# vfdev-5/interpolate-antialiasing

Hardware: AMD Instinct MI355X
Metric: Mpix/s (input pixels) antialiased bilinear 438x906->196x320, uint8 channels_last, PIL-exact (higher is better)
Workload: dtype u8; 1 GPU; uint8 channels_last [1024,3,438,906]->[196,320] bilinear antialias per GPU (BASELINE configs[1] batched), Pillow-exact integer arithmetic; batch_per_gpu=1024, global_batch=1024, variant=fused_u8_nhwc_pil_v3, parallelism=batch-shard x1, lib=interpolate_antialiasing_amd/csrc/libaa_interp.so

## Files before the change

interpolate_antialiasing_amd/csrc/aa_fused_u8_v3_impl.h:

```cpp

#pragma once
#include <math.h>
#include <stdio.h>
#include <stdlib.h>

#include <type_traits>

#include "aa_alpha.h"
#include "aa_plan.h"

#ifndef AA_V3_ABL
#define AA_V3_ABL 0
#endif

#ifndef AA_V3_AUX
#define AA_V3_AUX 0
#endif

#ifndef AA_V3_PRIO
#define AA_V3_PRIO 0
#endif
#ifndef AA_V3_DMA_EARLY
#define AA_V3_DMA_EARLY 0
#endif

#ifndef AA_V3_BURST
#define AA_V3_BURST 1
#endif

#ifndef AA_V3_F32OUT_AUX
#define AA_V3_F32OUT_AUX 0
#endif

#ifndef AA_V3_FLT_FAST
#define AA_V3_FLT_FAST 0
#endif

#ifndef AA_V3_UNALIGNED
#define AA_V3_UNALIGNED 0
#endif

struct FusedU8V3Params {
  int H, W, oH, oW;
  int ksize_w, ksize_h;
  int ybands, nstrips;
  int strips_per_block;
  int strip_w;
  int nseg;
  int seg_bytes;
  int sc_off;
  int gather_off;
  int in_mis;
  unsigned long long img_in_bytes, img_out_bytes, total_in_bytes, total_out_bytes;
  long long n_images;
  int spb_forced;
  int outm, normalize, cin;
  float mean[4], std[4];
  unsigned row_pitch;
  int fast;
  int byte_store;
  unsigned long long plane_in_bytes, plane_out_bytes;
  long long pl_planes;
  int out16, pair_store;
};

namespace {

typedef __attribute__((address_space(3))) void lds_void;

#ifndef AA_V3_STORE_AUX
#define AA_V3_STORE_AUX 2
#endif
constexpr int kStoreAuxInterleaved = AA_V3_STORE_AUX;




__device__ inline unsigned pack2_bf16(float lo, float hi) {
  unsigned d;
  asm("v_cvt_pk_bf16_f32 %0, %1, %2" : "=v"(d) : "v"(lo), "v"(hi));
  return d;
}
__device__ inline unsigned pack2_f16(float lo, float hi) {
  typedef _Float16 half2_t __attribute__((ext_vector_type(2)));
  const half2_t t = {(_Float16)lo, (_Float16)hi};
  return __builtin_bit_cast(unsigned, t);
}

__device__ inline float right_neighbour(float x) {
  return __int_as_float(__builtin_amdgcn_update_dpp(__float_as_int(x), __float_as_int(x), 0xF5 , 0xF, 0xF, false));
}

__device__ inline int clip8_int(int acc) {
  acc >>= 22;
  return acc < 0 ? 0 : (acc > 255 ? 255 : acc);
}

__device__ inline void wait_vmcnt(int n) {
  if (n >= 12) { asm volatile("s_waitcnt vmcnt(12)" ::: "memory"); return; }
  if (n >= 8) { asm volatile("s_waitcnt vmcnt(8)" ::: "memory"); return; }
  if (n >= 6) { asm volatile("s_waitcnt vmcnt(6)" ::: "memory"); return; }
  if (n >= 4) { asm volatile("s_waitcnt vmcnt(4)" ::: "memory"); return; }
  if (n >= 3) { asm volatile("s_waitcnt vmcnt(3)" ::: "memory"); return; }
  if (n >= 2) { asm volatile("s_waitcnt vmcnt(2)" ::: "memory"); return; }
  if (n >= 1) { asm volatile("s_waitcnt vmcnt(1)" ::: "memory"); return; }
  asm volatile("s_waitcnt vmcnt(0)" ::: "memory");
}

#ifndef AA_V3_WAVES_PER_EU
#define AA_V3_WAVES_PER_EU 0
#endif
#if AA_V3_WAVES_PER_EU
#define AA_V3_OCC __attribute__((amdgpu_waves_per_eu(AA_V3_WAVES_PER_EU, AA_V3_WAVES_PER_EU)))
#else
#define AA_V3_OCC
#endif
template <int C, int TW, int G, bool TWO_DMA, int MAXC, bool NONNEG, bool PERIODIC, bool FLT = false, int UPK = 0, int PL = 0, int SP = 1,
          bool ALPHA = false, bool O16 = false>
__global__ void __launch_bounds__(512) AA_V3_OCC
fused_u8_nhwc_v3_kernel(const uint8_t *__restrict__ in, uint8_t *__restrict__ out, const char *__restrict__ tab_w,
                        const char *__restrict__ tab_h, const FusedU8V3Params p) {
  static_assert(PL == 0 || (PL == C && !PERIODIC && UPK == 0 && !TWO_DMA), "plane groups: shrinking heights, fixed stage layout");
  static_assert(SP == 1 || (SP == 4 && !FLT && !PERIODIC && UPK == 0 && PL == 0), "split windows: integer arithmetic, shrinking heights");
  static_assert(!ALPHA || (C == 4 && !FLT && PL == 0), "premultiplied alpha: Pillow arithmetic, 4 interleaved channels");
  static_assert(!O16 || (FLT && SP == 1), "16-bit float output: float arithmetic");
  constexpr int PLN = PL > 0 ? PL : 1;
  constexpr int CB = PL > 0 ? 1 : C;
  constexpr int NV1 = (CB * TW + 3) / 4;
  constexpr int ND1 = NV1 + 1;
  constexpr int NV = PLN * NV1, ND = PLN * ND1;
  struct SA { unsigned s[PLN]; };
  constexpr int PL_SLOT = 1024, PL_PIECES = 21, PL_PLANE = PL_PIECES * 16;
  extern __shared__ __attribute__((aligned(16))) uint8_t lds[];

  const int lane = threadIdx.x & 63;
  const int wv = __builtin_amdgcn_readfirstlane(threadIdx.x >> 6);
  const int sgroups = (p.nstrips + p.strips_per_block - 1) / p.strips_per_block;
  const int xcd = blockIdx.x & 7, k = blockIdx.x >> 3;
  const int strip = (k % sgroups) * p.strips_per_block + wv;
  const long long grp = (long long)(k / sgroups) * 8 + xcd;
  if (grp >= p.n_images * p.ybands) return;
  if (strip >= p.nstrips) return;
  const bool full_group = (k % sgroups + 1) * p.strips_per_block <= p.nstrips;
  const int yb = (int)(grp % p.ybands);
  const int n = (int)(grp / p.ybands);
  const int ox0 = strip * p.strip_w;
  const int bw = min(p.strip_w, p.oW - ox0);
  const int oy0 = (int)((long long)yb * p.oH / p.ybands);
  const int oy1 = (int)((long long)(yb + 1) * p.oH / p.ybands);

  const int32_t *__restrict__ xmin_w = (const int32_t *)(tab_w + aa_table_xmin_off());
  const int32_t *__restrict__ xsize_w = (const int32_t *)(tab_w + aa_table_xsize_off(p.oW));
  const int32_t *__restrict__ kw = (const int32_t *)(tab_w + aa_table_w_off(p.oW));
  const int32_t *__restrict__ ymin_h = (const int32_t *)(tab_h + aa_table_xmin_off());
  const int32_t *__restrict__ ysize_h = (const int32_t *)(tab_h + aa_table_xsize_off(p.oH));
  const int32_t *__restrict__ sc_rec = (const int32_t *)(tab_h + p.sc_off);
  const int32_t *__restrict__ g_rec = (const int32_t *)(tab_h + p.gather_off);

  const int r_begin = __builtin_amdgcn_readfirstlane(ymin_h[oy0]);
  const int ylm = __builtin_amdgcn_readfirstlane(ymin_h[oy1 - 1]);
  const int yls = __builtin_amdgcn_readfirstlane(ysize_h[oy1 - 1]);
  const int r_stop = ylm + (yls > 1 ? yls : 1);
  const int n_rows = r_stop - r_begin;
  const int n_groups = (n_rows + G - 1) / G;

  const int sp_px = SP > 1 ? lane / SP : lane;
  const int sp_part = SP > 1 ? lane % SP : 0;
  const bool active = sp_px < bw;
  const int ox = ox0 + (active ? sp_px : 0);
  const int xm = xmin_w[ox];
  int xs = xsize_w[ox];
  xs = xs > 1 ? xs : 1;
  int lead = xm + TW * SP - p.W;
  lead = lead > 0 ? lead : 0;
  const int start = xm - lead + sp_part * TW;
  const int acc_init = (SP > 1 && sp_part != 0) ? 0 : 1 << 21;
  int wreg[TW];
#pragma unroll
  for (int j = 0; j < TW; j++) {
    const int src = sp_part * TW + j - lead;
    int w = (src >= 0 && src < xs && src < p.ksize_w) ? kw[(size_t)ox * p.ksize_w + src] : 0;
    wreg[j] = FLT ? w : (w << 8) >> 8;
  }
  asm volatile("s_waitcnt vmcnt(0)" ::: "memory");
  const int seg_first = __builtin_amdgcn_readfirstlane(start * CB);
  const int c_l = start * CB - seg_first;

  const unsigned long long img_off = (unsigned long long)p.in_mis + (unsigned long long)n * p.img_in_bytes;
  const unsigned long long base_off = img_off & ~15ull;
  unsigned long long remaining = p.total_in_bytes - base_off;
  if constexpr (PL == 0) remaining = (remaining + 3ull) & ~3ull;
  if (remaining > 0xFFFFFFFCull) remaining = 0xFFFFFFFCull;
  const __amdgpu_buffer_rsrc_t rsrc =
      __builtin_amdgcn_make_buffer_rsrc((void *)(in + base_off), 0, (unsigned)remaining, 0x00020000);
  const unsigned row_bytes = p.row_pitch;
  const int lds_base = PL > 0 ? wv * G * PL_SLOT : wv * G * p.seg_bytes;
  const unsigned lane_lds = (unsigned)(lds_base + c_l);
  unsigned pl_voff = 0;
  bool pl_dma_lane = false;
  if constexpr (PL > 0) {
    const int pc = lane / PL_PIECES, piece = lane - pc * PL_PIECES;
    pl_voff = (unsigned)pc * (unsigned)p.plane_in_bytes + (unsigned)piece * 16u;
    pl_dma_lane = pc < PL && piece < p.nseg;
  }
  const bool dma_lane0 = PL > 0 ? pl_dma_lane : lane < p.nseg;
  const bool dma_lane1 = lane + 64 < p.nseg;
  constexpr int dma_per_row = TWO_DMA ? 2 : 1;
  const unsigned voff = (unsigned)lane * 16u;

  const unsigned long long out_off = (unsigned long long)n * p.img_out_bytes;
  unsigned long long out_rem = p.total_out_bytes - out_off;
  if (out_rem > 0xFFFFFFFFull) out_rem = 0xFFFFFFFFull;
  const __amdgpu_buffer_rsrc_t orsrc = __builtin_amdgcn_make_buffer_rsrc((void *)(out + out_off), 0, (unsigned)out_rem, 0x00020000);
  const unsigned out_row_bytes = (unsigned)p.oW * CB;
  const int pl_valid = PL > 0 ? (int)(p.pl_planes - (long long)n * PL < PL ? p.pl_planes - (long long)n * PL : PL) : C;
  float nm_mean[C], nm_std[C];
#pragma unroll
  for (int c = 0; c < C; c++) {
    const int ch = PL > 0 ? (int)(((long long)n * PL + c) % (p.cin > 0 ? p.cin : 1))
                          : (C == 1 ? (int)(n % (p.cin > 0 ? p.cin : 1)) : c);
    nm_mean[c] = FLT ? p.mean[ch & 3] : 0.f;
    nm_std[c] = FLT ? p.std[ch & 3] : 1.f;
  }
  unsigned store_voff;
  bool store_lane;
  unsigned perm_sel = 0;
  if constexpr (PL > 0) {
    store_voff = (unsigned)(ox0 + lane);
    store_lane = ((lane & 3) == 0) && ((lane | 3) < bw);
  } else if constexpr (C == 3) {
    const int q = lane & 3;
    store_voff = (unsigned)(ox0 * 3 + (lane >> 2) * 12 + q * 4);
    store_lane = (q != 3) && ((lane | 3) < bw);
    perm_sel = q == 0 ? 0x04020100u : (q == 1 ? 0x05040201u : 0x06050402u);
  } else if constexpr (C == 1) {
    store_voff = (unsigned)(ox0 + lane);
    store_lane = ((lane & 3) == 0) && ((lane | 3) < bw);
  } else {
    store_voff = (unsigned)((ox0 + lane) * 4);
    store_lane = active;
  }

  unsigned a = (unsigned)(img_off - base_off) + (unsigned)seg_first + (unsigned)r_begin * row_bytes;

  int A[MAXC][C];
#pragma unroll
  for (int k = 0; k < MAXC; k++)
#pragma unroll
    for (int c = 0; c < C; c++) A[k][c] = FLT ? 0 : 1 << 21;
  int o_base = oy0;

  constexpr int RK = UPK > 0 ? UPK : 1;
  int ring[RK][C];
#pragma unroll
  for (int k = 0; k < RK; k++)
#pragma unroll
    for (int c = 0; c < C; c++) ring[k][c] = 0;
  int vm_issued = 0, idxv = 0;

  auto dma = [&](unsigned a_row, int slot) {
    if (AA_V3_ABL == 4) return;
    if constexpr (UPK > 0) {
      vm_issued += TWO_DMA ? 2 : 1;
      idxv = (lane == slot) ? vm_issued : idxv;
    }
    if (AA_V3_PRIO) __builtin_amdgcn_s_setprio(3);
    const unsigned soff = AA_V3_ABL == 7 ? (a_row & 0x3F0u) : (a_row & ~15u);
    const int dst = lds_base + slot * (PL > 0 ? PL_SLOT : p.seg_bytes);
    if constexpr (PL > 0) {
      if (dma_lane0) __builtin_amdgcn_raw_ptr_buffer_load_lds(rsrc, (lds_void *)(lds + dst), 16, pl_voff, a_row, 0, AA_V3_AUX);
      if (AA_V3_PRIO) __builtin_amdgcn_s_setprio(0);
      return;
    }
    if (dma_lane0) __builtin_amdgcn_raw_ptr_buffer_load_lds(rsrc, (lds_void *)(lds + dst), 16, voff, soff, 0, AA_V3_AUX);
    if constexpr (TWO_DMA) {
      if (dma_lane1)
        __builtin_amdgcn_raw_ptr_buffer_load_lds(rsrc, (lds_void *)(lds + dst + 1024), 16, voff + 1024, soff, 0, AA_V3_AUX);
    }
    if (AA_V3_PRIO) __builtin_amdgcn_s_setprio(0);
  };
  unsigned slot_ra[G];
  unsigned slot_ph[G];
#pragma unroll
  for (int j = 0; j < G; j++) {
    const unsigned ph = (a + (unsigned)j * row_bytes) & 15u;
    slot_ph[j] = (unsigned)(j * p.seg_bytes) + ph;
    slot_ra[j] = (lane_lds + slot_ph[j]) & ~3u;
  }
  auto fetch = [&](unsigned a_row, int slot, unsigned (&d)[ND], bool tables = true) -> SA {
    SA r;
    unsigned sa, ra;
    if (AA_V3_ABL == 6) { for (int c = 0; c < PLN; c++) r.s[c] = 0; return r; }
    if constexpr (PL > 0) {
      const __attribute__((address_space(3))) unsigned *al = (const __attribute__((address_space(3))) unsigned *)(uintptr_t)(lane_lds & ~3u);
#pragma unroll
      for (int c = 0; c < PL; c++) {
#pragma unroll
        for (int k = 0; k < ND1; k++) d[c * ND1 + k] = al[(slot * PL_SLOT + c * PL_PLANE) / 4 + k];
        r.s[c] = lane_lds;
      }
      return r;
    }
    if (PERIODIC && tables) {
      sa = lane_lds + slot_ph[slot];
      ra = slot_ra[slot];
    } else {
      sa = lane_lds + (unsigned)(slot * p.seg_bytes) + (a_row & 15u);
      ra = sa & ~3u;
    }
    if constexpr (AA_V3_UNALIGNED) {
      typedef unsigned u32_any __attribute__((aligned(1)));
      const __attribute__((address_space(3))) u32_any *ul = (const __attribute__((address_space(3))) u32_any *)(uintptr_t)sa;
#pragma unroll
      for (int k = 0; k < NV; k++) d[k] = ul[k];
      d[ND - 1] = 0;
      r.s[0] = sa;
      return r;
    }
    const __attribute__((address_space(3))) unsigned *al = (const __attribute__((address_space(3))) unsigned *)(uintptr_t)ra;
#pragma unroll
    for (int k = 0; k < ND; k++) d[k] = al[k];
    r.s[0] = sa;
    return r;
  };
  struct Scatter { int first; int cc; int w[MAXC]; };
  auto load_scatter = [&](int r) -> Scatter {
    Scatter s;
    if constexpr (UPK > 0) {
      s.first = 0; s.cc = 0;
#pragma unroll
      for (int k = 0; k < MAXC; k++) s.w[k] = 0;
      return s;
    }
    const int32_t *rec = (const int32_t *)((const char *)sc_rec + (unsigned)r * 32u);
    s.first = __builtin_amdgcn_readfirstlane(rec[0]);
    s.cc = __builtin_amdgcn_readfirstlane(rec[1]);
#pragma unroll
    for (int k = 0; k < MAXC; k++) s.w[k] = __builtin_amdgcn_readfirstlane(rec[2 + k]);
    return s;
  };
  auto trunc8 = [&](int bits) -> unsigned {
    float a = __int_as_float(bits);
    a = a < 0.f ? 0.f : (a > 255.f ? 255.f : a);
    return (unsigned)(int)a;
  };
  const int emit_path = __builtin_amdgcn_readfirstlane(
      (FLT && p.outm != 0) ? (O16 ? (1 | (p.pair_store ? 2 : 0) | (p.out16 == 2 ? 4 : 0) | ((C == 1 || p.outm == 1) ? 8 : 0)) : 1) : (p.byte_store ? 2 : 0));
  auto emit = [&](int oy) {
    if constexpr (ALPHA) {
      const int al = clip8_int(A[0][3]);
#pragma unroll
      for (int c = 0; c < 3; c++) A[0][c] = aa_unpremul8(clip8_int(A[0][c]), al) << 22;
      A[0][3] = al << 22;
    }
    if constexpr (FLT) {
      if constexpr (O16) {
        if (emit_path & 1) {
          int lane_o = lane;
          asm volatile("" : "+v"(lane_o));
          auto pack2 = [&](float lo, float hi) -> unsigned { return (emit_path & 4) ? pack2_bf16(lo, hi) : pack2_f16(lo, hi); };
          auto value = [&](int c) -> float {
            const float x = __int_as_float(A[0][c]);
            return p.normalize ? (x - nm_mean[c]) / nm_std[c] : x;
          };
          const bool pairs = (emit_path & 2) != 0;
          const bool all = lane_o < bw, st = all && (!pairs || (lane_o & 1) == 0);
          if (emit_path & 8) {
            if constexpr (UPK > 0) vm_issued += C;
            const unsigned fv = (unsigned)(ox0 + lane_o) * 2u;
#pragma unroll
            for (int c = 0; c < C; c++) {
              const unsigned fs = ((unsigned)c * (unsigned)p.oH + (unsigned)oy) * (unsigned)p.oW * 2u;
              const float x = value(c);
              const unsigned d = pack2(x, right_neighbour(x));
              if (pairs) {
                if (st && (PL == 0 || c < pl_valid)) __builtin_amdgcn_raw_buffer_store_b32(d, orsrc, fv, fs, AA_V3_F32OUT_AUX);
              } else {
                if (st && (PL == 0 || c < pl_valid)) __builtin_amdgcn_raw_buffer_store_b16((unsigned short)d, orsrc, fv, fs, AA_V3_F32OUT_AUX);
              }
            }
          } else if constexpr (C > 1) {
            const unsigned fv = (unsigned)(ox0 + lane_o) * (unsigned)(2 * C), fs = (unsigned)oy * (unsigned)p.oW * (unsigned)(2 * C);
            float x[C];
#pragma unroll
            for (int c = 0; c < C; c++) x[c] = value(c);
            unsigned d[3];
            if constexpr (C == 3) {
              d[2] = pack2(right_neighbour(x[1]), right_neighbour(x[2]));
              d[1] = pack2(x[2], right_neighbour(x[0]));
              d[0] = pack2(x[0], x[1]);
            } else {
              d[0] = pack2(x[0], x[1]);
              d[1] = pack2(x[2], x[C - 1]);
              d[2] = 0;
            }
            if (!pairs) {
              if constexpr (UPK > 0) vm_issued += C;
#pragma unroll
              for (int c = 0; c < C; c++)
                if (all) __builtin_amdgcn_raw_buffer_store_b16((unsigned short)(d[c >> 1] >> (16 * (c & 1))), orsrc, fv + 2u * (unsigned)c, fs, AA_V3_F32OUT_AUX);
            } else {
              if constexpr (UPK > 0) vm_issued += 1;
              if constexpr (C == 3) {
                typedef unsigned u32x3 __attribute__((ext_vector_type(3)));
                const u32x3 t = {d[0], d[1], d[2]};
                if (st) __builtin_amdgcn_raw_buffer_store_b96(t, orsrc, fv, fs, AA_V3_F32OUT_AUX);
              } else {
                typedef unsigned u32x2 __attribute__((ext_vector_type(2)));
                const u32x2 t = {d[0], d[1]};
                if (all) __builtin_amdgcn_raw_buffer_store_b64(t, orsrc, fv, fs, AA_V3_F32OUT_AUX);
              }
            }
          }
        }
      } else
      if (emit_path == 1) {
        float v[C];
        int lane_o = lane;
        asm volatile("" : "+v"(lane_o));
#pragma unroll
        for (int c = 0; c < C; c++) {
          v[c] = __int_as_float(A[0][c]);
          if (p.normalize) v[c] = (v[c] - nm_mean[c]) / nm_std[c];
        }
        if (p.outm == 1) {
          if constexpr (UPK > 0) vm_issued += C;
#pragma unroll
          for (int c = 0; c < C; c++)
            if (active && (PL == 0 || c < pl_valid))
              __builtin_amdgcn_raw_buffer_store_b32(__float_as_uint(v[c]), orsrc, (unsigned)(ox0 + lane_o) * 4u,
                                                    ((unsigned)c * (unsigned)p.oH + (unsigned)oy) * (unsigned)p.oW * 4u, AA_V3_F32OUT_AUX);
        } else {
          if constexpr (UPK > 0) vm_issued += 1;
          const unsigned fv = (unsigned)(ox0 + lane_o) * (unsigned)(4 * C), fs = (unsigned)oy * (unsigned)p.oW * (unsigned)(4 * C);
          if constexpr (C == 3) {
            typedef unsigned u32x3 __attribute__((ext_vector_type(3)));
            const u32x3 t = {__float_as_uint(v[0]), __float_as_uint(v[1]), __float_as_uint(v[2])};
            if (active) __builtin_amdgcn_raw_buffer_store_b96(t, orsrc, fv, fs, AA_V3_F32OUT_AUX);
          } else if constexpr (C == 4) {
            typedef unsigned u32x4 __attribute__((ext_vector_type(4)));
            const u32x4 t = {__float_as_uint(v[0]), __float_as_uint(v[1]), __float_as_uint(v[2]), __float_as_uint(v[3])};
            if (active) __builtin_amdgcn_raw_buffer_store_b128(t, orsrc, fv, fs, AA_V3_F32OUT_AUX);
          } else {
            if (active) __builtin_amdgcn_raw_buffer_store_b32(__float_as_uint(v[0]), orsrc, fv, fs, AA_V3_F32OUT_AUX);
          }
        }
      }
    }
    if (emit_path == 2) {
      int lane_o = lane;
      asm volatile("" : "+v"(lane_o));
      const int px_o = SP > 1 ? lane_o / SP : lane_o;
      const unsigned bv = (unsigned)((ox0 + px_o) * CB);
      const bool act = px_o < bw && (SP == 1 || (lane_o % SP) == 0);
      if constexpr (UPK > 0) vm_issued += C;
#pragma unroll
      for (int c = 0; c < C; c++) {
        const unsigned b = FLT ? trunc8(A[0][c]) : (unsigned)clip8_int(A[0][c]);
        if constexpr (PL > 0) {
          if (act && c < pl_valid) __builtin_amdgcn_raw_buffer_store_b8((unsigned char)b, orsrc, bv, (unsigned)c * (unsigned)p.plane_out_bytes + (unsigned)oy * out_row_bytes, 0);
        } else {
          if (act) __builtin_amdgcn_raw_buffer_store_b8((unsigned char)b, orsrc, bv + c, (unsigned)oy * out_row_bytes, 0);
        }
      }
    }
    if constexpr (UPK > 0) {
      if (emit_path == 0) vm_issued += 1;
    }
    if (emit_path != 0) {
    } else if constexpr (PL > 0) {
      const unsigned t = FLT ? (trunc8(A[0][0]) | (trunc8(A[0][1]) << 8) | (trunc8(A[0][PL > 2 ? 2 : 1]) << 16))
                             : pack4_clip8(A[0][0], A[0][1], A[0][PL > 2 ? 2 : 1], A[0][PL - 1]);
      const unsigned nb = (unsigned)__builtin_amdgcn_update_dpp(0, (int)t, 0xF5 , 0xF, 0xF, false);
#pragma unroll
      for (int c = 0; c < PL; c++) {
        const unsigned pair = __builtin_amdgcn_perm(nb, t, 0x0c0c0000u | (unsigned)((4 + c) << 8) | (unsigned)c);
        const unsigned hi = (unsigned)__builtin_amdgcn_update_dpp(0, (int)pair, 0xAA , 0xF, 0xF, false);
        const unsigned dw = __builtin_amdgcn_perm(hi, pair, 0x05040100u);
        if (store_lane && c < pl_valid) __builtin_amdgcn_raw_buffer_store_b32(dw, orsrc, store_voff, (unsigned)c * (unsigned)p.plane_out_bytes + (unsigned)oy * out_row_bytes, 0);
      }
    } else if constexpr (C == 3) {
      const unsigned t = FLT ? (trunc8(A[0][0]) | (trunc8(A[0][1]) << 8) | (trunc8(A[0][2]) << 16))
                             : pack4_clip8(A[0][0], A[0][1], A[0][2], A[0][2]);
      const unsigned nb = (unsigned)__builtin_amdgcn_update_dpp(0, (int)t, 0xF9 , 0xF, 0xF, false);
      const unsigned dw = __builtin_amdgcn_perm(nb, t, perm_sel);
      if (store_lane && (AA_V3_ABL != 1 || dw == 0x12345678u))
        __builtin_amdgcn_raw_buffer_store_b32(dw, orsrc, store_voff, AA_V3_ABL == 9 ? 0u : (unsigned)oy * out_row_bytes, C == 1 ? 0 : kStoreAuxInterleaved);
    } else if constexpr (C == 1) {
      const unsigned t = FLT ? trunc8(A[0][0]) * 0x01010101u : pack4_clip8(A[0][0], A[0][0], A[0][0], A[0][0]);
      const unsigned n1 = (unsigned)__builtin_amdgcn_update_dpp(0, (int)t, 0x55 , 0xF, 0xF, false);
      const unsigned n2 = (unsigned)__builtin_amdgcn_update_dpp(0, (int)t, 0xAA , 0xF, 0xF, false);
      const unsigned n3 = (unsigned)__builtin_amdgcn_update_dpp(0, (int)t, 0xFF , 0xF, 0xF, false);
      const unsigned dw = (t & 0x000000ffu) | (n1 & 0x0000ff00u) | (n2 & 0x00ff0000u) | (n3 & 0xff000000u);
      if (store_lane) __builtin_amdgcn_raw_buffer_store_b32(dw, orsrc, store_voff, (unsigned)oy * out_row_bytes, C == 1 ? 0 : kStoreAuxInterleaved);
    } else {
      const unsigned dw = FLT ? (trunc8(A[0][0]) | (trunc8(A[0][1]) << 8) | (trunc8(A[0][2]) << 16) | (trunc8(A[0][C - 1]) << 24))
                              : pack4_clip8(A[0][0], A[0][1], A[0][2], A[0][C - 1]);
      if (store_lane) __builtin_amdgcn_raw_buffer_store_b32(dw, orsrc, store_voff, (unsigned)oy * out_row_bytes, C == 1 ? 0 : kStoreAuxInterleaved);
    }
#pragma unroll
    for (int k = 0; k + 1 < MAXC; k++)
#pragma unroll
      for (int c = 0; c < C; c++) A[k][c] = A[k + 1][c];
#pragma unroll
    for (int c = 0; c < C; c++) A[MAXC - 1][c] = FLT ? 0 : 1 << 21;
  };
  struct GRow { int m; int s; int w[RK]; };
  auto load_grow = [&](int oy) -> GRow {
    GRow gr;
    const int o = oy < p.oH ? oy : p.oH - 1;
    const int32_t *rec = (const int32_t *)((const char *)g_rec + (unsigned)o * 32u);
    gr.m = __builtin_amdgcn_readfirstlane(rec[0]);
    gr.s = __builtin_amdgcn_readfirstlane(rec[1]);
#pragma unroll
    for (int k = 0; k < RK; k++) gr.w[k] = __builtin_amdgcn_readfirstlane(rec[2 + (k < 6 ? k : 5)]);
    return gr;
  };
  GRow g_cur, g_nxt;
  if constexpr (UPK > 0) {
    g_cur = load_grow(oy0);
    g_nxt = load_grow(oy0 + 1);
  }
  int r = r_begin;
  auto realign = [&](const unsigned (&d)[ND], const SA &sa, unsigned (&v)[NV]) {
#pragma unroll
    for (int c = 0; c < PLN; c++)
#pragma unroll
      for (int k = 0; k < NV1; k++)
        v[c * NV1 + k] = AA_V3_UNALIGNED ? d[c * ND1 + k] : __builtin_amdgcn_alignbyte(d[c * ND1 + k + 1], d[c * ND1 + k], sa.s[c]);
  };
  bool steady = false;
  auto row_step = [&](const unsigned (&v)[NV], const Scatter &sc, auto steady_tag) {
    constexpr bool STEADY = decltype(steady_tag)::value;
    if (AA_V3_ABL == 6) return;
    int h[C];
    if constexpr (FLT) {
      float accf[C];
#pragma unroll
      for (int j = 0; j < TW; j++) {
#pragma unroll
        for (int c = 0; c < C; c++) {
          const int bi = PL > 0 ? c * (4 * NV1) + j : j * C + c;
          const float px = (float)((v[bi >> 2] >> (8 * (bi & 3))) & 0xffu);
          if constexpr (AA_V3_FLT_FAST != 0) {
            accf[c] = j == 0 ? px * __int_as_float(wreg[j]) : __builtin_fmaf(px, __int_as_float(wreg[j]), accf[c]);
            continue;
          }
          const float prod = px * __int_as_float(wreg[j]);
          accf[c] = j == 0 ? prod : accf[c] + prod;
        }
      }
#pragma unroll
      for (int c = 0; c < C; c++) h[c] = __float_as_int(accf[c]);
    } else {
      int acc[C];
#pragma unroll
      for (int c = 0; c < C; c++) acc[c] = AA_V3_ABL == 5 ? (int)v[c] : (SP > 1 ? acc_init : 1 << 21);
#pragma unroll
      for (int j = 0; j < (AA_V3_ABL == 5 ? 0 : TW); j++) {
#pragma unroll
        for (int c = 0; c < C; c++) {
          const int bi = PL > 0 ? c * (4 * NV1) + j : j * C + c;
          int px = (int)((v[bi >> 2] >> (8 * (bi & 3))) & 0xffu);
          if constexpr (ALPHA) {
            if (c < 3) px = aa_premul8(px, (int)(v[j] >> 24));
          }
          acc[c] += px * wreg[j];
        }
      }
      if constexpr (SP > 1) {
#pragma unroll
        for (int c = 0; c < C; c++) {
          acc[c] += __builtin_amdgcn_update_dpp(0, acc[c], 0xB1 , 0xF, 0xF, false);
          acc[c] += __builtin_amdgcn_update_dpp(0, acc[c], 0x4E , 0xF, 0xF, false);
        }
      }
#pragma unroll
      for (int c = 0; c < C; c++) h[c] = NONNEG ? (int)((unsigned)acc[c] >> 22) : clip8_int(acc[c]);
    }
    if constexpr (UPK > 0) {
#pragma unroll
      for (int k = 0; k + 1 < RK; k++)
#pragma unroll
        for (int c = 0; c < C; c++) ring[k][c] = ring[k + 1][c];
#pragma unroll
      for (int c = 0; c < C; c++) ring[RK - 1][c] = h[c];
      while (o_base < oy1) {
        int gs = g_cur.s > 1 ? g_cur.s : 1;
        if (g_cur.m + gs != r + 1) break;
        gs = gs < RK ? gs : RK;
#pragma unroll
        for (int ss = 1; ss <= RK; ss++) {
          if (gs == ss) {
#pragma unroll
            for (int c = 0; c < C; c++) {
              int acc;
              if constexpr (FLT) {
                float f = __int_as_float(ring[RK - ss][c]) * __int_as_float(g_cur.w[0]);
#pragma unroll
                for (int k2 = 1; k2 < ss; k2++) f = f + __int_as_float(ring[RK - ss + k2][c]) * __int_as_float(g_cur.w[k2]);
                acc = __float_as_int(f);
              } else {
                acc = (1 << 21) + __mul24(ring[RK - ss][c], g_cur.w[0]);
#pragma unroll
                for (int k2 = 1; k2 < ss; k2++) acc += __mul24(ring[RK - ss + k2][c], g_cur.w[k2]);
              }
              A[0][c] = acc;
            }
          }
        }
        emit(o_base);
        o_base++;
        g_cur = g_nxt;
        g_nxt = load_grow(o_base + 1);
      }
      return;
    }
    auto vmac = [&](int a, int hv, int w) -> int {
      if constexpr (FLT && AA_V3_FLT_FAST != 0) return __float_as_int(__builtin_fmaf(__int_as_float(hv), __int_as_float(w), __int_as_float(a)));
      else if constexpr (FLT) return __float_as_int(__int_as_float(a) + __int_as_float(hv) * __int_as_float(w));
      else return a + __mul24(hv, w);
    };
    const int idx0 = sc.first - o_base;
    if constexpr (STEADY) {
#pragma unroll
      for (int k = 0; k < MAXC; k++) {
        if (k >= 2 && k >= (sc.cc & 0xFFFF)) break;
#pragma unroll
        for (int c = 0; c < C; c++) A[k][c] = vmac(A[k][c], h[c], sc.w[k]);
      }
    } else if (__builtin_expect(idx0 == 0, 1)) {
      steady = true;
#pragma unroll
      for (int k = 0; k < MAXC; k++) {
        if (k >= 2 && k >= (sc.cc & 0xFFFF)) break;
#pragma unroll
        for (int c = 0; c < C; c++) A[k][c] = vmac(A[k][c], h[c], sc.w[k]);
      }
    } else if (idx0 < 0 && idx0 > -MAXC) {
#pragma unroll
      for (int s = 1; s < MAXC; s++) {
        if (idx0 == -s) {
#pragma unroll
          for (int k = s; k < MAXC; k++)
#pragma unroll
            for (int c = 0; c < C; c++) A[k - s][c] = vmac(A[k - s][c], h[c], sc.w[k]);
        }
      }
    }
    const int sc_end = sc.first + (sc.cc >> 16);
    const int e_end = sc_end < oy1 ? sc_end : oy1;
    while (o_base < e_end) {
      emit(o_base);
      o_base++;
    }
  };

  const int pl_fix_row = (PL > 0 && (long long)n + 1 == p.n_images) ? p.H - 1 : -1;
  auto pl_patch_last = [&](int slot) {
    if constexpr (PL > 0) {
      const int q = p.W - 3 + lane;
      const int lpos = q - seg_first;
      if (lane < 3 && q >= 0 && lpos >= 0 && lpos < p.nseg * 16) {
        const uint8_t b = in[img_off + (unsigned long long)(pl_valid - 1) * p.plane_in_bytes + (unsigned long long)(p.H - 1) * row_bytes + (unsigned)q];
        lds[lds_base + slot * PL_SLOT + (pl_valid - 1) * PL_PLANE + lpos] = b;
      }
      asm volatile("s_waitcnt vmcnt(0) lgkmcnt(0)" ::: "memory");
    }
  };

  for (int i = 0; i < G; i++)
    if (i < n_rows) dma(a + (unsigned)i * row_bytes, i);
  unsigned d0[ND], d1[ND];
  SA sa0 = {}, sa1 = {};
  Scatter sc0 = load_scatter(r_begin), sc1 = sc0;
  {
    const int younger = (n_rows < G ? n_rows : G) - 1;
    wait_vmcnt(younger * dma_per_row);
    if (PL > 0 && r_begin == pl_fix_row) pl_patch_last(0);
    sa0 = fetch(a, 0, d0, false);
  }
  for (int g = 0; g < n_groups; g++) {
    const int x0 = g * G;
    auto unrolled_group = [&](auto steady_tag) {
      if (full_group) __builtin_amdgcn_s_barrier();
#pragma unroll
      for (int i = 0; i < G; i++) {
        if (AA_V3_ABL != 2) asm volatile("s_waitcnt vmcnt(%0)" ::"n"(dma_per_row * (G - 2 - (i % AA_V3_BURST))) : "memory");
        unsigned v[NV];
        if ((i & 1) == 0) {
          realign(d0, sa0, v);
          __builtin_amdgcn_sched_barrier(0);
          sc1 = load_scatter(r + 1);
          sa1 = fetch(a + row_bytes, (i + 1) % G, d1);
          __builtin_amdgcn_sched_barrier(0);
          if (AA_V3_DMA_EARLY) { dma(a + (unsigned)G * row_bytes, i); __builtin_amdgcn_sched_barrier(0); }
          row_step(v, sc0, steady_tag);
        } else {
          realign(d1, sa1, v);
          __builtin_amdgcn_sched_barrier(0);
          sc0 = load_scatter(r + 1);
          sa0 = fetch(a + row_bytes, (i + 1) % G, d0);
          __builtin_amdgcn_sched_barrier(0);
          if (AA_V3_DMA_EARLY) { dma(a + (unsigned)G * row_bytes, i); __builtin_amdgcn_sched_barrier(0); }
          row_step(v, sc1, steady_tag);
        }
        if (!AA_V3_DMA_EARLY) {
          if constexpr (AA_V3_BURST == 1) {
            dma(a + (unsigned)G * row_bytes, i);
          } else if ((i % AA_V3_BURST) == AA_V3_BURST - 1) {
#pragma unroll
            for (int b = AA_V3_BURST - 1; b >= 0; b--) dma(a + (unsigned)(G - b) * row_bytes, i - b);
          }
        }
        a += row_bytes;
        r++;
        __builtin_amdgcn_sched_barrier(0);
      }
    };
    if (UPK == 0 && x0 + 2 * G <= n_rows) {
      if (steady) unrolled_group(std::true_type{});
      else unrolled_group(std::false_type{});
    } else {
      for (int i = 0; i < G; i++) {
        const int x = x0 + i;
        if (x >= n_rows) break;
        if (x + 1 < n_rows) {
          if constexpr (UPK > 0) {
            const int my_idx = __builtin_amdgcn_readlane(idxv, __builtin_amdgcn_readfirstlane((i + 1) % G));
            wait_vmcnt(vm_issued - my_idx);
          } else {
            int younger = n_rows - 1 - (x + 1);
            younger = younger < G - 2 ? younger : G - 2;
            wait_vmcnt(younger * dma_per_row);
          }
          if (PL > 0 && r + 1 == pl_fix_row) pl_patch_last((i + 1) % G);
          if ((i & 1) == 0) { sc1 = load_scatter(r + 1); sa1 = fetch(a + row_bytes, (i + 1) % G, d1, false); }
          else { sc0 = load_scatter(r + 1); sa0 = fetch(a + row_bytes, (i + 1) % G, d0, false); }
        }
        unsigned v[NV];
        if ((i & 1) == 0) { realign(d0, sa0, v); row_step(v, sc0, std::false_type{}); }
        else { realign(d1, sa1, v); row_step(v, sc1, std::false_type{}); }
        if (x + G < n_rows) dma(a + (unsigned)G * row_bytes, i);
        a += row_bytes;
        r++;
      }
    }
  }
}

int pick_ybands(int64_t items_per_band, double slots, int taps_h, int64_t H, int64_t oH) {
  const int64_t max_yb = oH / 8 > 1 ? oH / 8 : 1;
  int64_t ybands = 1;
  double best = 1e30;
  for (int64_t yb = 1; yb <= max_yb && yb <= 64; yb++) {
    const double rounds = (double)items_per_band * yb / slots;
    const double eff = rounds / ceil(rounds);
    const double halo = 1.0 + (double)(yb - 1) * taps_h / (double)H;
    const double cost = halo / eff;
    if (cost < best - 1e-9) {
      best = cost;
      ybands = yb;
    }
  }
  if (const char *e = aa_knob("AA_FUSED_YBANDS")) {
    const int64_t v = atoll(e);
    if (v >= 1 && v <= max_yb) ybands = v;
  }
  return (int)ybands;
}

template <int C, int TW, int G, int MAXC, bool TWO, bool NONNEG, bool PERIODIC, bool FLT = false, int UPK = 0, int PL = 0, int SP = 1,
          bool ALPHA = false, bool O16 = false>
int launch_k(FusedU8V3Params p, const AAProblem &q, size_t lds) {
  auto kern = fused_u8_nhwc_v3_kernel<C, TW, G, TWO, MAXC, NONNEG, PERIODIC, FLT, UPK, PL, SP, ALPHA, O16>;
  auto resident = [&](int s) {
    int nb = aa_resident_blocks(kern, 64 * s, lds * s);
    if (nb <= 0) nb = 16 / s;
    return nb < 1 ? 1 : nb;
  };
  int spb = p.strips_per_block;
  if (spb > 1 && !p.spb_forced && resident(1) > resident(spb) * spb) spb = 1;
  p.strips_per_block = spb;
  const int sgroups = (p.nstrips + spb - 1) / spb;
  const size_t lds_blk = lds * spb;
  const int taps_h = q.ah.max_taps > 0 ? q.ah.max_taps : q.ah.ksize;
  p.ybands = pick_ybands(p.n_images * sgroups, (double)aa_device_cu_count() * resident(spb), taps_h, q.H, q.oH);
  if (aa_knob("AA_V3_DEBUG"))
    fprintf(stderr, "[aa v3] strips %d spb %d (resident(1) %d, resident(%d) %d) ybands %d lds/strip %zu images %lld\n", p.nstrips, spb,
            resident(1), p.nstrips <= 8 ? p.nstrips : 4, resident(p.nstrips <= 8 ? p.nstrips : 4), p.ybands, lds, (long long)p.n_images);
  const int64_t groups8 = (p.n_images * (int64_t)p.ybands + 7) / 8 * 8;
  const int64_t grid = groups8 * sgroups;
  if (grid > 0x7FFFFFFF) return 0;
  hipLaunchKernelGGL(kern, dim3((unsigned)grid), dim3(64 * spb), lds_blk,
                     q.stream, (const uint8_t *)q.in - p.in_mis, (uint8_t *)q.out, (const char *)q.aw.table_dev,
                     (const char *)q.ah.table_dev, p);
  AA_HIP_CHECK_LAUNCH();
  return 1;
}

int round_tw(int taps) {
  const int opts[] = {2, 4, 6, 8, 12, 16, 24, 34};
  for (int o : opts)
    if (taps <= o) return o;
  return 0;
}

}

enum V3Route {
#define V3_ROUTE(route, ...) V3_##route,
#include "aa_fused_u8_v3_list.h"
};
enum V3Arith { V3_PIL = 1, V3_FLT = 2, V3_BOTH = 3 };
constexpr bool v3_route_has_out16(int route) { return route == V3_NARROW || route == V3_UP || route == V3_PLANES; }
```

Baseline: 1.429 million Mpix/s.

## Use 2D grid with magic division and defer weight-table waits in prologue

The block index mapping moves to a 2D grid: strip groups on x and image/band items on y, with a host-computed magic multiplier replacing the 64-bit divisions and modulos. Per-pixel weights are now loaded through a buffer resource without bounds branches. Masking and LDS offset computation are deferred until after the scatter load, so the table loads overlap with other setup instead of stalling on vmcnt(0) before the row DMAs are issued. The aim is a shorter kernel prologue, at the cost of more complex indexing and a host-side fallback check for magic-division validity.

```diff
diff --git a/interpolate_antialiasing_amd/csrc/aa_fused_u8_v3_impl.h b/interpolate_antialiasing_amd/csrc/aa_fused_u8_v3_impl.h
--- a/interpolate_antialiasing_amd/csrc/aa_fused_u8_v3_impl.h
+++ b/interpolate_antialiasing_amd/csrc/aa_fused_u8_v3_impl.h
@@ -62,6 +62,10 @@
   unsigned long long plane_in_bytes, plane_out_bytes;
   long long pl_planes;
   int out16, pair_store;
+  int geo;
+  int sgroups;
+  unsigned yb_magic;
+  unsigned n_items;
 };
 
 namespace {
@@ -135,19 +139,36 @@
 
   const int lane = threadIdx.x & 63;
   const int wv = __builtin_amdgcn_readfirstlane(threadIdx.x >> 6);
-  const int sgroups = (p.nstrips + p.strips_per_block - 1) / p.strips_per_block;
-  const int xcd = blockIdx.x & 7, k = blockIdx.x >> 3;
-  const int strip = (k % sgroups) * p.strips_per_block + wv;
-  const long long grp = (long long)(k / sgroups) * 8 + xcd;
-  if (grp >= p.n_images * p.ybands) return;
+  asm volatile("" ::"s"(p.W), "s"(p.oH), "s"(p.oW), "s"(p.ksize_w), "s"(p.ybands), "s"(p.nstrips),
+               "s"(p.strips_per_block), "s"(p.strip_w), "s"(p.nseg), "s"(p.seg_bytes), "s"(p.sc_off), "s"(p.in_mis), "s"(p.img_in_bytes),
+               "s"(p.img_out_bytes), "s"(p.total_in_bytes), "s"(p.total_out_bytes), "s"(p.row_pitch), "s"(p.byte_store), "s"(p.geo),
+               "s"(p.yb_magic), "s"(p.n_items));
+  const int xcd = blockIdx.x & 7;
+  int ks, yb, n, oy0, oy1;
+  if (p.geo) {
+    ks = blockIdx.x >> 3;
+    const unsigned g = blockIdx.y * 8u + (unsigned)xcd;
+    if (g >= p.n_items) return;
+    const bool one = p.ybands == 1;
+    n = (int)(one ? g : __umulhi(g, p.yb_magic));
+    yb = (int)(g - (unsigned)n * (unsigned)p.ybands);
+    oy0 = (int)(one ? 0u : __umulhi((unsigned)yb * (unsigned)p.oH, p.yb_magic));
+    oy1 = (int)(one ? (unsigned)p.oH : __umulhi((unsigned)(yb + 1) * (unsigned)p.oH, p.yb_magic));
+  } else {
+    const int k = blockIdx.x >> 3;
+    ks = k % p.sgroups;
+    const long long grp = (long long)(k / p.sgroups) * 8 + xcd;
+    if (grp >= p.n_images * p.ybands) return;
+    yb = (int)(grp % p.ybands);
+    n = (int)(grp / p.ybands);
+    oy0 = (int)((long long)yb * p.oH / p.ybands);
+    oy1 = (int)((long long)(yb + 1) * p.oH / p.ybands);
+  }
+  const int strip = ks * p.strips_per_block + wv;
   if (strip >= p.nstrips) return;
-  const bool full_group = (k % sgroups + 1) * p.strips_per_block <= p.nstrips;
-  const int yb = (int)(grp % p.ybands);
-  const int n = (int)(grp / p.ybands);
+  const bool full_group = (ks + 1) * p.strips_per_block <= p.nstrips;
   const int ox0 = strip * p.strip_w;
   const int bw = min(p.strip_w, p.oW - ox0);
-  const int oy0 = (int)((long long)yb * p.oH / p.ybands);
-  const int oy1 = (int)((long long)(yb + 1) * p.oH / p.ybands);
 
   const int32_t *__restrict__ xmin_w = (const int32_t *)(tab_w + aa_table_xmin_off());
   const int32_t *__restrict__ xsize_w = (const int32_t *)(tab_w + aa_table_xsize_off(p.oW));
@@ -168,23 +189,25 @@
   const int sp_part = SP > 1 ? lane % SP : 0;
   const bool active = sp_px < bw;
   const int ox = ox0 + (active ? sp_px : 0);
-  const int xm = xmin_w[ox];
+  const int xm_first = xmin_w[ox0], xm_last = xmin_w[ox0 + bw - 1];
+  int lead0 = xm_first + TW * SP - p.W;
+  lead0 = lead0 > 0 ? lead0 : 0;
+  const int seg_first = (xm_first - lead0) * CB;
+  int xm = xmin_w[ox];
   int xs = xsize_w[ox];
-  xs = xs > 1 ? xs : 1;
-  int lead = xm + TW * SP - p.W;
-  lead = lead > 0 ? lead : 0;
-  const int start = xm - lead + sp_part * TW;
+  const __amdgpu_buffer_rsrc_t wrsrc =
+      __builtin_amdgcn_make_buffer_rsrc((void *)kw, 0, (unsigned)(p.oW * p.ksize_w) * 4u, 0x00020000);
+  unsigned w_off = (unsigned)(ox * p.ksize_w + sp_part * TW) * 4u;
   const int acc_init = (SP > 1 && sp_part != 0) ? 0 : 1 << 21;
+  if (xm_last + TW * SP > p.W) {
+    const int lead_e = xm + TW * SP - p.W;
+    w_off -= (unsigned)(lead_e > 0 ? lead_e : 0) * 4u;
+    asm volatile("" : "+v"(w_off));
+  }
   int wreg[TW];
 #pragma unroll
-  for (int j = 0; j < TW; j++) {
-    const int src = sp_part * TW + j - lead;
-    int w = (src >= 0 && src < xs && src < p.ksize_w) ? kw[(size_t)ox * p.ksize_w + src] : 0;
-    wreg[j] = FLT ? w : (w << 8) >> 8;
-  }
-  asm volatile("s_waitcnt vmcnt(0)" ::: "memory");
-  const int seg_first = __builtin_amdgcn_readfirstlane(start * CB);
-  const int c_l = start * CB - seg_first;
+  for (int j = 0; j < TW; j++) wreg[j] = (int)__builtin_amdgcn_raw_buffer_load_b32(wrsrc, w_off + (unsigned)j * 4u, 0, 0);
+  __builtin_amdgcn_sched_barrier(0);
 
   const unsigned long long img_off = (unsigned long long)p.in_mis + (unsigned long long)n * p.img_in_bytes;
   const unsigned long long base_off = img_off & ~15ull;
@@ -195,7 +218,7 @@
       __builtin_amdgcn_make_buffer_rsrc((void *)(in + base_off), 0, (unsigned)remaining, 0x00020000);
   const unsigned row_bytes = p.row_pitch;
   const int lds_base = PL > 0 ? wv * G * PL_SLOT : wv * G * p.seg_bytes;
-  const unsigned lane_lds = (unsigned)(lds_base + c_l);
+  unsigned lane_lds = 0;
   unsigned pl_voff = 0;
   bool pl_dma_lane = false;
   if constexpr (PL > 0) {
@@ -285,8 +308,25 @@
   for (int j = 0; j < G; j++) {
     const unsigned ph = (a + (unsigned)j * row_bytes) & 15u;
     slot_ph[j] = (unsigned)(j * p.seg_bytes) + ph;
-    slot_ra[j] = (lane_lds + slot_ph[j]) & ~3u;
-  }
+    slot_ra[j] = 0;
+  }
+  auto tables_landed = [&]() {
+    xs = xs > 1 ? xs : 1;
+    int lead = xm + TW * SP - p.W;
+    lead = lead > 0 ? lead : 0;
+    const unsigned taps = (unsigned)(xs < p.ksize_w ? xs : p.ksize_w);
+#pragma unroll
+    for (int j = 0; j < TW; j++) {
+      const int src = sp_part * TW + j - lead;
+      const int w = (unsigned)src < taps ? wreg[j] : 0;
+      wreg[j] = FLT ? w : (w << 8) >> 8;
+    }
+    const int start = xm - lead + sp_part * TW;
+    lane_lds = (unsigned)(lds_base + start * CB - seg_first);
+#pragma unroll
+    for (int j = 0; j < G; j++) slot_ra[j] = (lane_lds + slot_ph[j]) & ~3u;
+    __builtin_amdgcn_sched_barrier(0);
+  };
   auto fetch = [&](unsigned a_row, int slot, unsigned (&d)[ND], bool tables = true) -> SA {
     SA r;
     unsigned sa, ra;
@@ -669,14 +709,20 @@
     }
   };
 
-  for (int i = 0; i < G; i++)
-    if (i < n_rows) dma(a + (unsigned)i * row_bytes, i);
+  Scatter sc0 = load_scatter(r_begin), sc1 = sc0;
+  tables_landed();
+  if (n_rows >= G) {
+#pragma unroll
+    for (int i = 0; i < G; i++) dma(a + (unsigned)i * row_bytes, i);
+    asm volatile("s_waitcnt vmcnt(%0)" ::"n"((G - 1) * dma_per_row) : "memory");
+  } else {
+    for (int i = 0; i < G; i++)
+      if (i < n_rows) dma(a + (unsigned)i * row_bytes, i);
+    wait_vmcnt((n_rows - 1) * dma_per_row);
+  }
   unsigned d0[ND], d1[ND];
   SA sa0 = {}, sa1 = {};
-  Scatter sc0 = load_scatter(r_begin), sc1 = sc0;
   {
-    const int younger = (n_rows < G ? n_rows : G) - 1;
-    wait_vmcnt(younger * dma_per_row);
     if (PL > 0 && r_begin == pl_fix_row) pl_patch_last(0);
     sa0 = fetch(a, 0, d0, false);
   }
@@ -789,10 +835,24 @@
   if (aa_knob("AA_V3_DEBUG"))
     fprintf(stderr, "[aa v3] strips %d spb %d (resident(1) %d, resident(%d) %d) ybands %d lds/strip %zu images %lld\n", p.nstrips, spb,
             resident(1), p.nstrips <= 8 ? p.nstrips : 4, resident(p.nstrips <= 8 ? p.nstrips : 4), p.ybands, lds, (long long)p.n_images);
-  const int64_t groups8 = (p.n_images * (int64_t)p.ybands + 7) / 8 * 8;
+  const int64_t n_items = p.n_images * (int64_t)p.ybands;
+  const int64_t groups8 = (n_items + 7) / 8 * 8;
   const int64_t grid = groups8 * sgroups;
   if (grid > 0x7FFFFFFF) return 0;
-  hipLaunchKernelGGL(kern, dim3((unsigned)grid), dim3(64 * spb), lds_blk,
+  p.sgroups = sgroups;
+  p.n_items = (unsigned)n_items;
+  p.yb_magic = 0;
+  bool geo = groups8 / 8 <= 65535 && n_items <= 0x7FFFFFFF;
+  if (geo && p.ybands > 1) {
+    const uint64_t d = (uint64_t)p.ybands, M = ((1ull << 32) + d - 1) / d, e = M * d - (1ull << 32);
+    const uint64_t rows = d * (uint64_t)p.oH, xmax = (uint64_t)n_items > rows ? (uint64_t)n_items : rows;
+    geo = xmax < (1ull << 32) && xmax * e < (1ull << 32);
+    p.yb_magic = (unsigned)M;
+  }
+  if (const char *e = aa_knob("AA_V3_GEO")) geo = geo && atoi(e) != 0;
+  p.geo = geo ? 1 : 0;
+  const dim3 blocks = geo ? dim3(8u * (unsigned)sgroups, (unsigned)(groups8 / 8)) : dim3((unsigned)grid);
+  hipLaunchKernelGGL(kern, blocks, dim3(64 * spb), lds_blk,
                      q.stream, (const uint8_t *)q.in - p.in_mis, (uint8_t *)q.out, (const char *)q.aw.table_dev,
                      (const char *)q.ah.table_dev, p);
   AA_HIP_CHECK_LAUNCH();
```

Result: no change. 1.431 million Mpix/s (median of 3 runs) (+0.1%).
